# FerrisMind/candle-video

Measured on AMD Instinct MI355X. Metric: frames/sec end-to-end LTX-Video-2B 512x768x97; DiT step ms; VAE decode ms, higher is better.
Workload: dtype bf16; 1 GPU; LTX-Video-0.9.8-2B-distilled 512x768x97, 7 steps (configs.rs:223-240), untiled VAE decode; preset=0.9.8-2b-distilled, denoise_steps=7, parallelism=replicas x1 (no data-path collective)

## Files before the change

### candle-video_amd/csrc/capi_ops.hip

```cpp
#include "conv3d.h"
#include "../../include/ltxhip_ops.h"
#include "../../include/ltxhip_upsampler_st.h"
#include "../../include/ltxhip_stg.h"

static inline int dtc(int d) { return d == 1 ? LTX_DT_BF16 : LTX_DT_F32; }

extern "C" int ltx_op_linear(const void* x, const void* w, const void* bias, void* y, int M, int N, int K, int dtype, int epi,
                             const void* resid, const float* gate, int rows_per_batch, ltx_stream stream) {
    if (!x || !w || !y) LTX_FAIL(LTX_ERR_ARG, "ltx_op_linear: null tensor");
    if (epi < 0 || epi > 3) LTX_FAIL(LTX_ERR_ARG, "ltx_op_linear: epi must be 0..3");
    if ((epi == 2 || epi == 3) && !resid) LTX_FAIL(LTX_ERR_ARG, "ltx_op_linear: residual epilogue needs resid");
    if (epi == 2 && (!gate || rows_per_batch < 1)) LTX_FAIL(LTX_ERR_ARG, "ltx_op_linear: gated epilogue needs gate");
    GemmArgs g; g.A = x; g.W = w; g.C = y; g.bias = bias; g.resid = resid; g.gate = gate;
    g.M = M; g.N = N; g.K = K; g.lda = K; g.ldc = N; g.ldr = N; g.rows_per_batch = rows_per_batch > 0 ? rows_per_batch : 1; g.gate_stride = N;
    return ltx_launch_gemm(g, dtc(dtype), epi, (hipStream_t)stream);
}

extern "C" int64_t ltx_op_ring_packed_bytes(int N, int K) { return (int64_t)ltx_ring_packed_bytes(N, K); }
extern "C" int ltx_op_ring_pack(const void* w, int N, int K, void* out, ltx_stream stream) { return ltx_pack_ring_weights(w, N, K, out, (hipStream_t)stream); }
extern "C" int ltx_op_linear_packed(const void* x, const void* w, const void* w_packed, const void* bias, void* y, int M, int N, int K, int epi,
                                    const void* resid, const float* gate, int rows_per_batch, ltx_stream stream) {
    if (!x || !w || !w_packed || !y) LTX_FAIL(LTX_ERR_ARG, "ltx_op_linear_packed: null tensor");
    if (epi < 0 || epi > 3) LTX_FAIL(LTX_ERR_ARG, "ltx_op_linear_packed: epi must be 0..3");
    if ((epi == 2 || epi == 3) && !resid) LTX_FAIL(LTX_ERR_ARG, "ltx_op_linear_packed: residual epilogue needs resid");
// ... 305 lines not shown
        a.B = B; a.Sq = Sq; a.Sk = Sk; a.heads = heads; a.hd = 64; a.scale = scale; a.bias = (const float*)bc; a.k_count = (const int*)cnt;
        a.p_out = p_out; a.ldp = heads * KP;
        if (q_rowsq) { a.q_rowsq = q_rowsq; a.q_rowsq_n = q_rowsq_n; a.q_rowsq_D = D; a.q_rowsq_eps = q_rowsq_eps; }
        rc = ltx_launch_attention(a, LTX_DT_BF16, s);
    }
    if (rc == LTX_OK && counts_out && hipMemcpyAsync(counts_out, cnt, (size_t)B * 4, hipMemcpyDeviceToDevice, s) != hipSuccess) rc = LTX_ERR_HIP;
    const hipError_t e = hipStreamSynchronize(s);
    free_all();
    if (rc != LTX_OK) return rc;
    if (e != hipSuccess) { ltx_set_error(hipGetErrorString(e)); return LTX_ERR_HIP; }
    return LTX_OK;
}

extern "C" int ltx_op_attention_prescaled(const void* q, const void* k, const void* v, void* o, int B, int Sq, int Sk, int heads, int hd,
                                          int ldq, int ldk, int ldv, int ldo, ltx_stream stream) {
    if (!q || !k || !v || !o) LTX_FAIL(LTX_ERR_ARG, "ltx_op_attention_prescaled: null tensor");
    AttnArgs a; a.q = q; a.k = k; a.v = v; a.o = o; a.ldq = ldq; a.ldk = ldk; a.ldv = ldv; a.ldo = ldo;
    a.B = B; a.Sq = Sq; a.Sk = Sk; a.heads = heads; a.hd = hd; a.scale = 1.0f; a.q_prescaled = 1;
    return ltx_launch_attention(a, LTX_DT_BF16, (hipStream_t)stream);
}

namespace {
int conv_common(const void* x, const void* w, const void* bias, int wdtype, void* y, const void* resid,
                int B, int T, int H, int W, int Cin, int Cout, int causal, int dtype, int epi, int mode, int post, hipStream_t s, const PostNorm* pn = nullptr) {
    if (!x || !w || !bias || !y) LTX_FAIL(LTX_ERR_ARG, "conv: null tensor");
    const int dt = dtc(dtype), pad_t = causal ? 2 : 1;
    const Dims d{B, T, H, W};
    ConvW cw; cw.cin = Cin; cw.cout = Cout;
    if (pn) {
        if (B < 1 || T < 1 || H < 1 || W < 1 || Cin < 1 || Cout < 1) LTX_FAIL(LTX_ERR_ARG, "conv: empty problem");
        ConvW raw = cw; raw.w = const_cast<void*>(w); raw.b = const_cast<void*>(bias);
        GemmArgs g = conv_args(raw, d, pad_t, epi, pn); g.A = x; g.C = y;
        GemmRoute r;
        LTX_TRY(ltx_gemm_route(g, dt, epi, nullptr, false, &r));
        if (const char* why = ltx_gemm_route_refusal(g, r)) LTX_FAIL(LTX_ERR_ARG, why);
    }
    return conv3d_unpacked(dt, pad_t, cw, w, bias, dtc(wdtype), mode, x, y, d, epi, resid, post, s, pn);
}
}

extern "C" int ltx_op_conv3d(const void* x, const void* w, const void* bias, int wdtype, void* y, const void* resid,
                             int B, int T, int H, int W, int Cin, int Cout, int causal, int dtype, ltx_stream stream) {
    return conv_common(x, w, bias, wdtype, y, resid, B, T, H, W, Cin, Cout, causal, dtype, resid ? EPI_RESID : EPI_BIAS, LTX_PERM_NONE, 0, (hipStream_t)stream);
}
extern "C" int ltx_op_conv3d_norm(const void* x, const void* w, const void* bias, int wdtype, void* y, const float* scale, const float* shift, int mod_stride,
                                  float eps, int act, int B, int T, int H, int W, int Cin, int Cout, int causal, int dtype, ltx_stream stream) {
    if ((scale == nullptr) != (shift == nullptr)) LTX_FAIL(LTX_ERR_ARG, "ltx_op_conv3d_norm: scale and shift come together (both null: no modulation)");
    if (scale && mod_stride < Cout) LTX_FAIL(LTX_ERR_ARG, "ltx_op_conv3d_norm: mod_stride is the row stride of scale / shift, at least Cout");
    if (act != 0 && act != 1) LTX_FAIL(LTX_ERR_ARG, "ltx_op_conv3d_norm: act must be 0 (none) or 1 (SiLU)");
    if (!(eps >= 0.f)) LTX_FAIL(LTX_ERR_ARG, "ltx_op_conv3d_norm: eps must not be negative");
    PostNorm pn; pn.on = 1; pn.eps = eps; pn.act = act; pn.scale = scale; pn.shift = shift; pn.mod_stride = scale ? mod_stride : 0;
    return conv_common(x, w, bias, wdtype, y, nullptr, B, T, H, W, Cin, Cout, causal, dtype, EPI_BIAS, LTX_PERM_NONE, 0, (hipStream_t)stream, &pn);
}
extern "C" int ltx_op_upsample3d(const void* x, const void* w, const void* bias, int wdtype, void* y,
                                 int B, int T, int H, int W, int Cin, int Cout, int causal, int residual, int dtype, ltx_stream stream) {
    if (Cout % 8 != 0 || Cin % 8 != 0) LTX_FAIL(LTX_ERR_ARG, "upsample3d: channels must be multiples of 8");
    return conv_common(x, w, bias, wdtype, y, residual ? x : nullptr, B, T, H, W, Cin, Cout, causal, dtype, EPI_D2S, LTX_PERM_D2S, 0, (hipStream_t)stream);
}
extern "C" int ltx_op_conv3d_shuffle(const void* x, const void* w, const void* bias, int wdtype, void* y,
                                     int B, int F, int H, int W, int Cin, int O, int st, int ss, int dtype, ltx_stream stream) {
    if (!x || !w || !bias || !y) LTX_FAIL(LTX_ERR_ARG, "ltx_op_conv3d_shuffle: null tensor");
    if (!((st == 2 && ss == 1) || (st == 2 && ss == 2) || (st == 1 && ss == 2))) LTX_FAIL(LTX_ERR_ARG, "ltx_op_conv3d_shuffle: the factors (st, ss) are (2,1), (2,2) or (1,2)");
    if ((dtype != 0 && dtype != 1) || (wdtype != 0 && wdtype != 1)) LTX_FAIL(LTX_ERR_ARG, "ltx_op_conv3d_shuffle: bad dtype");
    const int nsub = st * ss * ss;
    if (B < 1 || F < 1 || H < 1 || W < 1 || F > (1 << 29) || H > (1 << 29) || W > (1 << 29)) LTX_FAIL(LTX_ERR_ARG, "ltx_op_conv3d_shuffle: bad shape");
    if (Cin < 8 || Cin % 8 != 0 || O < 4 * nsub || O % (4 * nsub) != 0) LTX_FAIL(LTX_ERR_ARG, "ltx_op_conv3d_shuffle: Cin must be a multiple of 8 and O a multiple of 4 x the sub-pixel count");
    if ((int64_t)B * (2 * F + 1) * (2 * H) * (2 * W) * std::max(Cin, O) > (1LL << 40)) LTX_FAIL(LTX_ERR_ARG, "ltx_op_conv3d_shuffle: shape too large");
    ConvW cw; cw.cin = Cin; cw.cout = O; cw.nsub = nsub;
    return conv3d_unpacked(dtc(dtype), 1, cw, w, bias, dtc(wdtype), LTX_PERM_D2S, x, y, Dims{B, F + 2, H, W}, EPI_D2S_G, nullptr, 0, (hipStream_t)stream);
}
extern "C" int ltx_op_conv_out_unpatchify(const void* x, const void* w, const void* bias, int wdtype, float* y,
                                          int B, int T, int H, int W, int Cin, int Cout, int causal, int postprocess, int dtype, ltx_stream stream) {
    if (Cout % 16 != 0) LTX_FAIL(LTX_ERR_ARG, "conv_out: Cout must be a multiple of 16 (patch 4x4)");
    return conv_common(x, w, bias, wdtype, y, nullptr, B, T, H, W, Cin, Cout, causal, dtype, EPI_UNPATCH, LTX_PERM_UNPATCH, postprocess, (hipStream_t)stream);
}

extern "C" int ltx_op_blend(const float* a, float* b, int BC, int at, int ah, int aw, int bt, int bh, int bw, int dim, int blend_extent, ltx_stream stream) {
    if (!a || !b || dim < 2 || dim > 4) LTX_FAIL(LTX_ERR_ARG, "ltx_op_blend: bad argument");
    const int ad[3] = {at, ah, aw}, bd[3] = {bt, bh, bw};
    BlendArgs ba; ba.a = a; ba.b = b; ba.dst = b; ba.BC = BC;
// ... 57 lines not shown
```

### candle-video_amd/csrc/conv_halo.hip

```cpp
#include <type_traits>
#include "gemm_common.h"
#include "options.h"

#ifndef HALO_WIDE_EPI
#define HALO_WIDE_EPI 1
#endif
#ifndef HALO_LOADERS
#define HALO_LOADERS 4
#endif
#ifndef HALO_PABL
#define HALO_PABL 0
#endif
#ifndef HALO_ABL
#define HALO_ABL 0
#endif

#ifdef HALO_TRACE
__device__ unsigned long long g_halo_trace[16384 * 8];
extern "C" int ltx_dbg_halo_trace(unsigned long long* out, int n) { return hipMemcpyFromSymbol(out, HIP_SYMBOL(g_halo_trace), (size_t)n * 8) == hipSuccess ? 0 : -1; }
#define HSTAMP(i) do { if (threadIdx.x == 0 && blockIdx.x < 16384) g_halo_trace[blockIdx.x * 8 + (i)] = __builtin_amdgcn_s_memrealtime(); } while (0)
#define HCYC(i) do { if (threadIdx.x == 0 && blockIdx.x < 16384) g_halo_trace[blockIdx.x * 8 + (i)] = __builtin_amdgcn_s_memtime(); } while (0)
#else
#define HSTAMP(i) do { } while (0)
#define HCYC(i) do { } while (0)
#endif

namespace {

constexpr int ROWB = 128;
constexpr int PH = 16, PW = 16, HW = PW + 2, HROWS = (PH + 2) * HW;
constexpr int A_PIECES = (HROWS + 7) / 8;
constexpr int A_STAGE = A_PIECES * 1024;
constexpr uint32_t OOB = 0x80000000u;
template <int I, int N, typename F> __device__ __forceinline__ void sfor_h(F&& f) {
    if constexpr (I < N) { f(std::integral_constant<int, I>{}); sfor_h<I + 1, N>(f); }
}

__device__ __forceinline__ int swz_h(int row, int chunk) { return row * ROWB + ((chunk ^ ((row >> 1) & 7)) << 4); }

extern __shared__ __attribute__((aligned(16))) unsigned char halo_smem[];

template <int BN, int WGM, int WGN, int EPI, bool PIPE>
__global__ __launch_bounds__(WGM * WGN * 64) void conv_halo_kernel(const GemmArgs g) {
    constexpr int NW = WGM * WGN, BM = PH * PW, WM = BM / WGM, WN = BN / WGN, FM = WM / 16, FN = BN == 64 ? 3 : WN / 16;
    static_assert((NW == 8 || (NW == 4 && PIPE)) && WM % 16 == 0 && WN % 16 == 0, "wave layout");
    constexpr int NTHR = NW * 64;
    constexpr int NL = (HALO_LOADERS == 4 && (BN == 128 || (BN == 64 && PIPE))) ? 4 : NW;
    constexpr int AJ = (A_PIECES + NL - 1) / NL, BJ = BN / (8 * NL);
    constexpr int B_STAGE = BN * ROWB;
    constexpr int A_ST = PIPE ? AJ * NL * 1024 : A_STAGE;
    static_assert(!PIPE || (NL == 4 && (BN == 128 || BN == 64)), "pipelined form: four loader waves, 128-wide tile (or conv_out's 64-wide one)");
    unsigned char* Abuf = halo_smem;
    unsigned char* Bbuf = halo_smem + 2 * A_ST;
    HSTAMP(0);
#ifndef HALO_NO_KERNARG_BATCH
    asm volatile("" :: "s"(g.A), "s"(g.W), "s"(g.C), "s"(g.bias), "s"(g.resid), "s"(g.N), "s"(g.K), "s"(g.Cin), "s"(g.T), "s"(g.H), "s"(g.Wd), "s"(g.ntaps), "s"(g.pad_t),
                 "s"(g.ldc), "s"(g.ldr), "s"(gridDim.x));
#endif

    const int tid = threadIdx.x, lane = tid & 63, wave = __builtin_amdgcn_readfirstlane(tid >> 6);
    const int wm = wave / WGN, wn = wave % WGN;
    const int lwave = wave & (NL - 1);
    const bool loader = wave < NL;
// ... 277 lines not shown
#pragma unroll
            for (int fm = 0; fm < FM; ++fm) {
                if (fm + 1 < FM) __builtin_amdgcn_sched_group_barrier(0x100, 1, 0);
                __builtin_amdgcn_sched_group_barrier(0x008, FN, 0);
            }
        }
        asm volatile("s_waitcnt vmcnt(0)" ::: "memory");
        __syncthreads();
    };
    for (int grp = 0; grp < G; ++grp) {
        const int p = grp & 1;
        step(grp, std::integral_constant<int, 0>{}, p);
        step(grp, std::integral_constant<int, 1>{}, p ^ 1);
        step(grp, std::integral_constant<int, 2>{}, p);
        step(grp, std::integral_constant<int, 3>{}, p ^ 1);
        step(grp, std::integral_constant<int, 4>{}, p);
        step(grp, std::integral_constant<int, 5>{}, p ^ 1);
        step(grp, std::integral_constant<int, 6>{}, p);
        step(grp, std::integral_constant<int, 7>{}, p ^ 1);
        step(grp, std::integral_constant<int, 8>{}, p);
    }

    }
    constexpr bool WIDE = HALO_WIDE_EPI && (EPI == EPI_BIAS || EPI == EPI_RESID);
    if constexpr (WIDE) {
        if (g.wide_epi) {
            constexpr int CPR = BN / 8, XM = 15, RPP = 64 / CPR;
            const int64_t frame_row0 = ((int64_t)b * g.T + t) * g.H * g.Wd;
            const __amdgpu_buffer_rsrc_t rr = __builtin_amdgcn_make_buffer_rsrc(
                const_cast<bf16_t*>(reinterpret_cast<const bf16_t*>(g.resid ? g.resid : g.C) + frame_row0 * g.ldr), 0, (int)OOB, 0x00020000);
            auto row_m = [&](int row, bool& inside) {
                const int y = y0 + (row >> 4), x = x0 + (row & 15);
                inside = y < g.H && x < g.Wd;
                return ((b * g.T + t) * g.H + y) * g.Wd + x;
            };
            if constexpr (EPI == EPI_RESID) {
                for (int pi = wave; pi < BM / RPP; pi += NW) {
                    const int row = pi * RPP + lane / CPR, pc = lane % CPR;
                    const int lc = pc ^ (row & XM);
                    bool inside; const int m = row_m(row, inside);
                    dma(rr, inside ? (uint32_t)((((int64_t)m - frame_row0) * g.ldr + n0 + lc * 8) * 2) : OOB, 0u, halo_smem + pi * 1024);
                }
                asm volatile("s_waitcnt vmcnt(0)" ::: "memory");
            }
            float bias4[FN][4];
#pragma unroll
            for (int fn = 0; fn < FN; ++fn) {
#pragma unroll
                for (int i = 0; i < 4; ++i) bias4[fn][i] = 0.f;
            }
// ... 18 lines not shown
                        float r[4];
                        load4<bf16_t>(reinterpret_cast<const bf16_t*>(slot), r);
#pragma unroll
                        for (int i = 0; i < 4; ++i) v[i] += r[i];
                    }
                    store4<bf16_t>(reinterpret_cast<bf16_t*>(slot), v);
                }
            }
            __syncthreads();
            bf16_t* Cb = reinterpret_cast<bf16_t*>(g.C);
            float pn_sc[8], pn_sh[8];
            bool pn_mod = false;
            if constexpr (EPI == EPI_BIAS) {
                if (g.pn_on && g.pn_scale) {
                    pn_mod = true;
                    const int c0 = tid % CPR;
                    const f32x4* scp = reinterpret_cast<const f32x4*>(g.pn_scale + (int64_t)b * g.pn_mod_stride + c0 * 8);
                    const f32x4* shp = reinterpret_cast<const f32x4*>(g.pn_shift + (int64_t)b * g.pn_mod_stride + c0 * 8);
                    const f32x4 s0 = scp[0], s1 = scp[1], h0 = shp[0], h1 = shp[1];
#pragma unroll
                    for (int j = 0; j < 4; ++j) { pn_sc[j] = 1.0f + s0[j]; pn_sc[4 + j] = 1.0f + s1[j]; pn_sh[j] = h0[j]; pn_sh[4 + j] = h1[j]; }
                }
            }
            for (int id = tid; id < BM * CPR; id += NTHR) {
                const int row = id / CPR, c = id - row * CPR;
                bool inside; const int m = row_m(row, inside);
                Chunk16 cc; cc.u = *reinterpret_cast<const u32x4*>(halo_smem + row * (CPR * 16) + ((c ^ (row & XM)) << 4));
                if constexpr (EPI == EPI_BIAS) {
                    if (g.pn_on) {
                        float f[8]; chunk_to_f32<bf16_t>(cc, f);
                        float ss = 0.f;
#pragma unroll
                        for (int j = 0; j < 8; ++j) ss += f[j] * f[j];
#pragma unroll
                        for (int o = CPR / 2; o > 0; o >>= 1) ss += __shfl_xor(ss, o);
                        const float rinv = __builtin_amdgcn_rsqf(ss * (1.0f / (float)BN) + g.pn_eps);
#pragma unroll
                        for (int j = 0; j < 8; ++j) {
                            float n = f[j] * rinv;
                            if (pn_mod) n = n * pn_sc[j] + pn_sh[j];
                            if (g.pn_act == 1) n = silu_f(n);
                            f[j] = n;
                        }
                        f32_to_chunk<bf16_t>(f, cc);
                    }
                }
                if (!inside) continue;
                *reinterpret_cast<u32x4*>(Cb + (int64_t)m * g.ldc + n0 + c * 8) = cc.u;
            }
#ifdef HALO_TRACE
            HSTAMP(3); asm volatile("s_waitcnt vmcnt(0)" ::: "memory"); HSTAMP(4);
            if (threadIdx.x == 0 && blockIdx.x < 16384) { unsigned hw; asm volatile("s_getreg_b32 %0, hwreg(HW_REG_HW_ID)" : "=s"(hw)); g_halo_trace[blockIdx.x * 8 + 7] = hw; }
#endif
            return;
        }
    }
    if constexpr (EPI == EPI_S2D) {
        float bias4[FN][4];
#pragma unroll
        for (int fn = 0; fn < FN; ++fn) {
#pragma unroll
            for (int i = 0; i < 4; ++i) bias4[fn][i] = 0.f;
        }
        if (g.bias) {
#pragma unroll
            for (int fn = 0; fn < FN; ++fn) {
                int nb = n0 + wn * WN + fn * 16 + 4 * fq; nb = nb < g.N ? nb : g.N - 4;
                load4<bf16_t>(reinterpret_cast<const bf16_t*>(g.bias) + nb, bias4[fn]);
            }
        }
        const int npass = (t == 0 && g.s2_st > 1) ? 2 : 1;
        for (int pass = 0; pass < npass; ++pass) {
// ... 18 lines not shown
                    for (int i = 0; i < 4; ++i) v[i] = acc[fm][fn][i] + bias4[fn][i];
                    s2d_store<bf16_t>(g, b, t, y, x, nb, pass, v, res[fn]);
                }
            }
        }
    } else if constexpr (EPI == EPI_D2S || EPI == EPI_UNPATCH || EPI == EPI_BIAS || EPI == EPI_D2S_G) {
        float bias4[FN][4];
#pragma unroll
        for (int fn = 0; fn < FN; ++fn) {
            const int nb = n0 + wn * WN + fn * 16 + 4 * fq;
#pragma unroll
            for (int i = 0; i < 4; ++i) bias4[fn][i] = 0.f;
        }
        if (g.bias) {
#pragma unroll
            for (int fn = 0; fn < FN; ++fn) {
                int nb = n0 + wn * WN + fn * 16 + 4 * fq; nb = nb < g.N ? nb : g.N - 4;
                load4<bf16_t>(reinterpret_cast<const bf16_t*>(g.bias) + nb, bias4[fn]);
            }
        }
        const bool d2s_res = EPI == EPI_D2S && g.resid != nullptr;
        GemmArgs gs = g; gs.bias = nullptr; gs.resid = nullptr;
        constexpr int FC = FM * FN > 16 ? 2 : FM;
#pragma unroll
        for (int f0 = 0; f0 < FM; f0 += FC) {
            bf16_t raw[FC][FN][4];
            if constexpr (EPI == EPI_D2S) {
                if (d2s_res) {
                    const int nsub = g.d2s_sp ? 4 : 8;
#pragma unroll
                    for (int fc = 0; fc < FC; ++fc) {
                        int y = y0 + wm * FM + f0 + fc, x = x0 + frow;
                        y = y < g.H ? y : g.H - 1; x = x < g.Wd ? x : g.Wd - 1;
                        const int m = ((b * g.T + t) * g.H + y) * g.Wd + x;
                        const bf16_t* xr = reinterpret_cast<const bf16_t*>(g.resid) + (int64_t)m * g.Cin;
#pragma unroll
                        for (int fn = 0; fn < FN; ++fn) {
                            int nb = n0 + wn * WN + fn * 16 + 4 * fq; nb = nb < g.N ? nb : g.N - 4;
                            const int sidx = nb / g.Cf, co = nb - sidx * g.Cf;
#pragma unroll
                            for (int i = 0; i < 4; ++i) raw[fc][fn][i] = xr[((co + i) % g.Cr) * nsub + sidx];
                        }
                    }
                }
            }
#pragma unroll
            for (int fc = 0; fc < FC; ++fc) {
                const int fm = f0 + fc;
                const int y = y0 + wm * FM + fm, x = x0 + frow;
                if (y >= g.H || x >= g.Wd) continue;
                const int m = ((b * g.T + t) * g.H + y) * g.Wd + x;
#pragma unroll
                for (int fn = 0; fn < FN; ++fn) {
                    const int nb = n0 + wn * WN + fn * 16 + 4 * fq;
                    if (nb >= g.N) continue;
                    float v[4];
#pragma unroll
                    for (int i = 0; i < 4; ++i) v[i] = acc[fm][fn][i] + bias4[fn][i];
                    if constexpr (EPI == EPI_D2S) {
                        if (d2s_res) {
#pragma unroll
                            for (int i = 0; i < 4; ++i) v[i] += to_f32(raw[fc][fn][i]);
                        }
                    }
                    epilogue<bf16_t, EPI>(gs, m, nb, v);
                }
            }
        }
    } else {
#pragma unroll
    for (int fm = 0; fm < FM; ++fm) {
        const int y = y0 + wm * FM + fm, x = x0 + frow;
        if (y >= g.H || x >= g.Wd) continue;
        const int m = ((b * g.T + t) * g.H + y) * g.Wd + x;
#pragma unroll
        for (int fn = 0; fn < FN; ++fn) {
            const int nb = n0 + wn * WN + fn * 16 + 4 * fq;
            if (nb >= g.N) continue;
            float v[4] = {acc[fm][fn][0], acc[fm][fn][1], acc[fm][fn][2], acc[fm][fn][3]};
            epilogue<bf16_t, EPI>(g, m, nb, v);
        }
    }
    }
}

bool halo_wide_epi(const GemmArgs& g) {
    return ltx_opt().gemm_wide_epi && g.ldc % 8 == 0 && ((uintptr_t)g.C & 15) == 0 &&
           (!g.resid || (g.ldr % 8 == 0 && ((uintptr_t)g.resid & 15) == 0 && (double)g.H * g.Wd * g.ldr * 2.0 < 2147483648.0));
}

template <int BN, int WGM, int WGN, int EPI, bool PIPE = false>
int launch_halo(const GemmArgs& g, hipStream_t s) {
    constexpr int smem = PIPE ? 2 * 44 * 1024 + 3 * BN * ROWB : 2 * A_STAGE + 2 * BN * ROWB;
    static std::atomic<unsigned long long> attr_devs{0};
    auto kern = conv_halo_kernel<BN, WGM, WGN, EPI, PIPE>;
    LTX_TRY(ltx_set_max_dyn_smem(attr_devs, reinterpret_cast<const void*>(kern), smem));
    const int tiles = g.B * g.T * cdiv(g.H, PH) * cdiv(g.Wd, PW) * cdiv(g.N, BN);
    GemmArgs ga = g;
    ga.wide_epi = halo_wide_epi(g);
    if (g.pn_on && (!ga.wide_epi || BN != g.N || !ltx_conv_halo_norm_ok(g, EPI))) LTX_FAIL(LTX_ERR_ARG, "conv_halo: the fused output norm needs the wide bias epilogue and BN == N");
    LTX_LAUNCH_TIMED(kern, dim3((unsigned)tiles), dim3(WGM * WGN * 64), smem, s, ga);
    LTX_CHECK_LAUNCH();
    return LTX_OK;
}

template <int BN, int WGM, int WGN, bool PIPE = false>
int launch_halo_epi(const GemmArgs& g, int epi, hipStream_t s) {
    switch (epi) {
        case EPI_BIAS: return launch_halo<BN, WGM, WGN, EPI_BIAS, PIPE>(g, s);
        case EPI_RESID: return launch_halo<BN, WGM, WGN, EPI_RESID, PIPE>(g, s);
        case EPI_D2S: return launch_halo<BN, WGM, WGN, EPI_D2S, PIPE>(g, s);
        case EPI_S2D: return launch_halo<BN, WGM, WGN, EPI_S2D, PIPE>(g, s);
        case EPI_D2S_G: return launch_halo<BN, WGM, WGN, EPI_D2S_G, PIPE>(g, s);
    }
    LTX_FAIL(LTX_ERR_ARG, "conv_halo: unsupported epilogue");
}

}

bool ltx_conv_halo_eligible(const GemmArgs& g, int epi, int bn) {
    if (!g.conv || g.ntaps != 27 || g.kh != 3 || g.kw != 3) return false;
    if (g.Cin % 64 != 0 || g.K != g.Cin) return false;
// ... 38 lines not shown
```

### candle-video_amd/csrc/options.cpp

```cpp
#include "options.h"
#include <atomic>
#include <cstdio>
#include <cstdlib>
#include <cstring>
#include <map>
#include <mutex>
#include <string>
#include "errors.h"

namespace {
std::mutex g_mu;
LtxOptions g_opt;
std::atomic<bool> g_loaded{false};
std::map<std::string, int> g_exp;

struct ListBit { const char* name; unsigned bit; };
const ListBit kFam[] = {{"asm16", LTX_FAM_ASM16}, {"ring", LTX_FAM_RING}, {"p8", LTX_FAM_P8}, {"halo", LTX_FAM_HALO}, {"halo_out", LTX_FAM_HALO_OUT}, {"big", LTX_FAM_BIG}};
const ListBit kAttn[] = {{"q64", LTX_ATTN_Q64}, {"q128", LTX_ATTN_Q128}, {"cross", LTX_ATTN_CROSS}, {"pipe", LTX_ATTN_PIPE}};

template <size_t N> bool parse_list(const char* v, const ListBit (&tab)[N], unsigned* out) {
    unsigned bits = 0;
    std::string s(v ? v : "");
    size_t p = 0;
    while (p < s.size()) {
        size_t q = s.find('+', p); if (q == std::string::npos) q = s.size();
        const std::string item = s.substr(p, q - p);
        bool ok = item.empty();
        for (const auto& t : tab) if (item == t.name) { bits |= t.bit; ok = true; }
        if (!ok) return false;
        p = q + 1;
    }
    *out = bits;
    return true;
}

struct IntField { const char* name; int LtxOptions::*field; };
const IntField kInts[] = {
    {"gemm_tune", &LtxOptions::gemm_tune}, {"gemm_wide_epi", &LtxOptions::gemm_wide_epi}, {"gemm_trace", &LtxOptions::gemm_trace},
    {"attn_q64_big", &LtxOptions::attn_q64_big}, {"vae_tile_batch", &LtxOptions::vae_tile_batch}, {"prof_kernel_events", &LtxOptions::prof_kernel_events}, {"ff2_defer", &LtxOptions::ff2_defer},
    {"gemm_splitk", &LtxOptions::gemm_splitk}, {"q2_fold", &LtxOptions::q2_fold}, {"norm_presum", &LtxOptions::norm_presum}, {"norm_lean", &LtxOptions::norm_lean},
    {"xattn_compact", &LtxOptions::xattn_compact}, {"xattn_fold_vo", &LtxOptions::xattn_fold_vo}, {"dense_qkv", &LtxOptions::dense_qkv}, {"vae_fuse_norm", &LtxOptions::vae_fuse_norm}, {"t5_attn_mfma", &LtxOptions::t5_attn_mfma}, {"guidance_batch", &LtxOptions::guidance_batch}, {"norm_fold", &LtxOptions::norm_fold}, {"norm_fold_copies", &LtxOptions::norm_fold_copies}, {"attn_q64_stream", &LtxOptions::attn_q64_stream},
};

bool set_one(LtxOptions& o, const std::string& key, const char* value) {
    static const LtxOptions dflt;
    for (const auto& f : kInts) if (key == f.name) {
        if (!value) { o.*(f.field) = dflt.*(f.field); return true; }
        char* end = nullptr; const long v = strtol(value, &end, 10);
        if (end == value || *end) return false;
        o.*(f.field) = (int)v; return true;
    }
    if (key == "gemm_plan") {
        if (!value) { o.gemm_plan[0] = 0; return true; }
        if (strlen(value) >= sizeof(o.gemm_plan)) return false;
        strcpy(o.gemm_plan, value); return true;
    }
    if (key == "gemm_off") return value ? parse_list(value, kFam, &o.gemm_off) : (o.gemm_off = 0, true);
    if (key == "attn_off") return value ? parse_list(value, kAttn, &o.attn_off) : (o.attn_off = 0, true);
    if (key.rfind("x_", 0) == 0) {
        if (!value) { g_exp.erase(key); return true; }
        char* end = nullptr; const long v = strtol(value, &end, 10);
// ... 81 lines not shown
```

### candle-video_amd/csrc/options.h

```cpp
#pragma once

enum { LTX_FAM_ASM16 = 1, LTX_FAM_RING = 2, LTX_FAM_P8 = 4, LTX_FAM_HALO = 8, LTX_FAM_HALO_OUT = 16, LTX_FAM_BIG = 32 };
enum { LTX_ATTN_Q64 = 1, LTX_ATTN_Q128 = 2, LTX_ATTN_CROSS = 4, LTX_ATTN_PIPE = 8 };

struct LtxOptions {
    int gemm_tune = 1;
    char gemm_plan[40] = {0};
    unsigned gemm_off = 0;
    int gemm_wide_epi = 1;
    int gemm_trace = 0;
    int attn_q64_big = -1;
    int vae_tile_batch = 0;
    int prof_kernel_events = 1;
    int ff2_defer = 1;
    int gemm_splitk = 1;
    int q2_fold = 1;
    int norm_presum = 1;
    int norm_lean = 1;
    int xattn_compact = 1;
    int xattn_fold_vo = 1;
    int attn_q64_stream = 0;
    int norm_fold = 2;
    int norm_fold_copies = 10;
    int guidance_batch = 1;
    int dense_qkv = 1;
    int vae_fuse_norm = 1;
    int t5_attn_mfma = 1;
    unsigned attn_off = 0;
};

const LtxOptions& ltx_opt();
int ltx_exp_lookup(const char* name, int dflt);
// ... 6 lines not shown
```

### candle-video_amd/ltxhip/__init__.py

```python
from __future__ import annotations

import ctypes as C
import os
from dataclasses import dataclass, field
from typing import Dict, List, Optional, Sequence, Tuple

import torch

_HERE = os.path.dirname(os.path.abspath(__file__))
_LIB_PATH = os.environ.get("LTXHIP_LIB") or os.path.join(os.path.dirname(_HERE), "libltxhip.so")

if not os.path.exists(_LIB_PATH):
    raise ImportError(
        f"ltxhip: {_LIB_PATH} is missing — build it with `make -C candle-video_amd` "
        "(or `python -c 'import __graft_entry__ as g; g.build()'`). There is no CPU fallback.")
lib = C.CDLL(_LIB_PATH)

LTX_F32, LTX_BF16 = 0, 1


class LtxError(RuntimeError):
    pass


# ... 85 lines not shown
    "ltx_op_linear_fold_out": [_vp, _vp, _vp, _vp, _vp, _vp, _vp, _i, _i, _i, _i, _i, _vp, _vp, _i, _vp],
    "ltx_op_linear_fold_in": [_vp, _vp, _vp, _vp, _i, _i, _f, _vp, _i, _i, _i, _i, _i, _i, _vp],
    "ltx_op_linear_fold_ok": [_i, _i, _i, _i, _i, _i, _i, _i],
    "ltx_op_shift_gemv": [_vp, _vp, _vp, _i, _i, _i, _i, _vp, _i, _vp],
    "ltx_op_mod_scale": [_vp, _vp, _i, _vp, _i, _i64, _i, _i, _vp], "ltx_op_scale_cols": [_vp, _vp, _vp, _i64, _i, _i, _vp],
    "ltx_op_linear_split_factor": [_i, _i, _i], "ltx_op_linear_deferred": [_vp, _vp, _vp, _i, _i, _i, _vp],
    "ltx_op_rownorm_deferred": [_vp, _i, _vp, _vp, _vp, _i, _vp, _vp, _i64, _i, _i, _f, _vp, _vp, _i64, _i, _i, _vp],
    "ltx_op_attention_compact": [_vp, _vp, _vp, _vp, _i, _i, _i, _i, _i, _i, _i, _i, _i, _f, _vp, _vp, _i, _i, _f, _vp, _vp],
    "ltx_op_attention_rowsq": [_vp, _vp, _vp, _vp, _i, _i, _i, _i, _i, _i, _i, _i, _i, _f, _vp, _vp, _i, _i, _f, _vp],
    "ltx_op_rownorm": [_vp, _vp, _i64, _i, _i, _f, _vp, _vp, _vp, _i64, _i, _i, _i, _vp],
    "ltx_op_qknorm_rope": [_vp, _i64, _i, _i, _vp, _f, _vp, _vp, _i, _vp],
    "ltx_op_qknorm_rope_segs": [_vp, _i64, _i, _i, _i, _i64, _vp, _vp, _vp, _f, _vp, _vp, _f, _i, _vp],
    "ltx_op_xattn_fold_route": [_i, _i, _i, _i, _i, _i, _i, C.POINTER(C.c_int)], "ltx_op_xattn_fold_kp": [C.POINTER(C.c_int), _i, C.POINTER(C.c_int)],
    "ltx_op_xattn_fold_build": [_vp, _vp, _vp, _i, _i, _i, _i, _vp, _vp, _vp],
    "ltx_op_attention_probs": [_vp, _vp, _vp, _i, _i, _i, _i, _i, _f, _vp, _vp, _i, _f, _vp, _vp],
    "ltx_op_norm_route": [_i64, _i, _i, _i, _i, _i, _i64, _i, _i, C.c_char_p, _i], "ltx_op_qknorm_route": [_i64, _i, _i, C.c_char_p, _i],
    "ltx_op_rope_table": [_vp, _vp, _vp, _i, _i, _i, _i, _i, _vp, _vp],
    "ltx_op_timestep_embedding": [_vp, _i, _i, _f, _i, _vp, _vp],
    "ltx_op_attention": [_vp, _vp, _vp, _vp, _i, _i, _i, _i, _i, _i, _i, _i, _i, _f, _vp, _i, _vp],
    "ltx_op_attention_prescaled": [_vp, _vp, _vp, _vp, _i, _i, _i, _i, _i, _i, _i, _i, _i, _vp],
    "ltx_op_conv3d": [_vp, _vp, _vp, _i, _vp, _vp, _i, _i, _i, _i, _i, _i, _i, _i, _vp],
    "ltx_op_conv3d_norm": [_vp, _vp, _vp, _i, _vp, _vp, _vp, _i, _f, _i, _i, _i, _i, _i, _i, _i, _i, _i, _vp],
    "ltx_op_upsample3d": [_vp, _vp, _vp, _i, _vp, _i, _i, _i, _i, _i, _i, _i, _i, _i, _vp],
    "ltx_op_conv_out_unpatchify": [_vp, _vp, _vp, _i, _vp, _i, _i, _i, _i, _i, _i, _i, _i, _i, _vp],
    "ltx_op_blend": [_vp, _vp, _i, _i, _i, _i, _i, _i, _i, _i, _i, _vp],
    "ltx_op_downsample3d": [_vp, _vp, _vp, _i, _vp, _i, _i, _i, _i, _i, _i, _i, _i, _vp],
    "ltx_op_gemm_plan": [_i, _i, _i, _i, _i, _i, _i, _i, C.c_char_p, _i],
    "ltx_op_gemm_route": [_i, _i, _i, _i, _i, _i, _i, _i, _i, _i, _i, _i, C.c_char_p, _i],
    "ltx_op_dit_plan": [_i, _i, _i, _i, _i, _i, _i, _i, _i, C.POINTER(C.c_int64)],
    "ltx_t5_config_default": [_vp], "ltx_t5_create": [_vp, _vp, _sz, _i, _i, _vp], "ltx_t5_destroy": [_vp],
    "ltx_t5_forward": [_vp, _vp, _i, _i, _i, _vp, _vp],
    "ltx_t5_create_from_gguf": [_vp, C.c_char_p, _i, _i, _vp], "ltx_t5_forward_masked": [_vp, _vp, _vp, _i, _i, _i, _vp, _vp],
    "ltx_gguf_open": [C.c_char_p, _vp], "ltx_gguf_close": [_vp], "ltx_gguf_count": [_vp], "ltx_gguf_find": [_vp, C.c_char_p],
    "ltx_gguf_tensor": [_vp, _sz, _vp, _vp, _vp, _vp, _vp, _vp], "ltx_gguf_type_info": [_i, _vp, _vp],
    "ltx_gguf_dequantize": [_i, _vp, _i, _i64, _i, _vp, _vp],
    "ltx_video_to_rgb8": [_vp, _i, _i, _i, _i, _vp, _vp], "ltx_write_png": [C.c_char_p, _vp, _i, _i],
    "ltx_save_frames_png": [_vp, _i, _i, _i, _i, C.c_char_p, _vp, _vp],
    "ltx_write_gif": [C.c_char_p, _vp, _i, _i, _i, _i, _i], "ltx_save_video_gif": [_vp, _i, _i, _i, _i, C.c_char_p, _vp],
    "ltx_preset_count": [], "ltx_preset_name": [_i], "ltx_preset_get": [C.c_char_p, _vp], "ltx_pipeline_params_from_preset": [_vp, _vp],
    "ltx_weights_detect_format": [C.c_char_p], "ltx_weights_remap_key": [C.c_char_p, C.c_char_p, _sz],
    "ltx_weights_is_transformer_key": [C.c_char_p], "ltx_weights_is_vae_key": [C.c_char_p],
    "ltx_name_mapper_create": [], "ltx_name_mapper_destroy": [_vp], "ltx_name_mapper_add": [_vp, _i, C.c_char_p, C.c_char_p],
    "ltx_name_mapper_has_mapping": [_vp, C.c_char_p], "ltx_name_mapper_map": [_vp, C.c_char_p, C.c_char_p, _sz],
    "ltx_weights_validate_names": [_vp, _sz, _vp, _sz, _vp, _vp],
    "ltx_safetensors_open": [C.c_char_p, _vp], "ltx_safetensors_close": [_vp], "ltx_safetensors_count": [_vp],
    "ltx_safetensors_tensor": [_vp, _sz, _vp, _vp, _vp, _vp, _vp, _vp],
# ... 1988 lines not shown
        ms = 0
        if scale is not None:
            for t in (scale, shift):
                if t.dtype != torch.float32 or tuple(t.shape) != (B, Cout) or t.stride(1) != 1:
                    raise LtxError(f"conv3d_norm: scale / shift must be f32 [{B}, {Cout}] with dense rows")
            ms = scale.stride(0) if B > 1 else max(scale.stride(0), Cout)
            if B > 1 and shift.stride(0) != ms:
                raise LtxError("conv3d_norm: scale and shift must share one row stride")
        y = torch.empty(B, T, H, W, Cout, dtype=x_cl.dtype, device=x_cl.device)
        _check(lib.ltx_op_conv3d_norm(_ptr(x_cl.contiguous()), _ptr(w.contiguous()), _ptr(bias.to(w.dtype).contiguous()), _dt(w.dtype), _ptr(y),
                                      _ptr(scale), _ptr(shift), ms, C.c_float(eps), act, B, T, H, W, Cin, Cout, int(causal), _dt(x_cl.dtype), _stream()))
        return y

    @staticmethod
    def upsample3d(x_cl, w, bias, causal=False, residual=True):
        B, T, H, W, Cin = x_cl.shape
        Cout = w.shape[0]
        y = torch.empty(B, 2 * T - 1, 2 * H, 2 * W, Cout // 8, dtype=x_cl.dtype, device=x_cl.device)
        _check(lib.ltx_op_upsample3d(_ptr(x_cl.contiguous()), _ptr(w.contiguous()), _ptr(bias.to(w.dtype).contiguous()), _dt(w.dtype), _ptr(y),
                                     B, T, H, W, Cin, Cout, int(causal), int(residual), _dt(x_cl.dtype), _stream()))
        return y

    @staticmethod
    def conv3d_shuffle(x_cl, w, bias, st, ss, out=None):
        x = x_cl.contiguous()
        B, Ft, H, W, Cin = x.shape
        F = Ft - 2
        O = w.shape[0]
        nsub = st * ss * ss
        shape = (B, (2 * F - 1 if st == 2 else F) + 2, ss * H, ss * W, O // max(nsub, 1))
        if out is None:
            out = torch.empty(shape, dtype=x.dtype, device=x.device)
        elif tuple(out.shape) != shape or out.dtype != x.dtype or not out.is_contiguous():
            raise LtxError(f"conv3d_shuffle: out must be a contiguous {shape} tensor of the input's dtype")
        _check(lib.ltx_op_conv3d_shuffle(_ptr(x), _ptr(w.contiguous()), _ptr(bias.to(w.dtype).contiguous()), _dt(w.dtype), _ptr(out),
                                         B, F, H, W, Cin, O, int(st), int(ss), _dt(x.dtype), _stream()))
        return out

    @staticmethod
    def pixel_shuffle_guarded(x_cl, out=None):
        x = x_cl.contiguous()
        B, Ft, H, W, C4 = x.shape
        if out is None:
            out = torch.empty(B, Ft, 2 * H, 2 * W, C4 // 4, dtype=x.dtype, device=x.device)
        _check(lib.ltx_op_pixel_shuffle_guarded(_ptr(x), _ptr(out), B, Ft - 2, H, W, C4 // 4, _dt(x.dtype), _stream()))
        return out
# ... 82 lines not shown
```

### include/ltxhip_ops.h

```cpp
#ifndef LTXHIP_OPS_H
#define LTXHIP_OPS_H
#include "ltxhip.h"
#ifdef __cplusplus
extern "C" {
#endif

int ltx_op_linear(const void* x, const void* w, const void* bias, void* y, int M, int N, int K, int dtype, int epi,
                  const void* resid, const float* gate, int rows_per_batch, ltx_stream stream);

int64_t ltx_op_ring_packed_bytes(int N, int K);
int ltx_op_ring_pack(const void* w, int N, int K, void* out, ltx_stream stream);
int ltx_op_linear_packed(const void* x, const void* w, const void* w_packed, const void* bias, void* y, int M, int N, int K, int epi,
                         const void* resid, const float* gate, int rows_per_batch, ltx_stream stream);
int ltx_op_linear_rowsq(const void* x, const void* w, const void* bias, void* y, float* rowsq, int M, int N, int K, int dtype, int epi,
                        const void* resid, const float* gate, int rows_per_batch, ltx_stream stream);
int ltx_op_rowsq(const void* x, int64_t rows, int N, int ld, float* rowsq, int dtype, ltx_stream stream);

int ltx_op_linear_fold_out(const void* x, const void* w, const void* bias, void* y, void* y2, float* rowsq, const float* scale2, int scale2_stride,
                           int M, int N, int K, int epi, const void* resid, const float* gate, int rows_per_batch, ltx_stream stream);
int ltx_op_linear_fold_in(const void* x, const void* w, void* y, const float* rs_sq, int rs_n, int rs_D, float eps, const float* cvec, int cvec_stride,
                          int M, int N, int K, int epi, int rows_per_batch, ltx_stream stream);
int ltx_op_linear_fold_ok(int M, int N, int K, int epi, int consumer, int rs_n, int vec_stride, int rows_per_batch);
int ltx_op_shift_gemv(const void* w, const void* bias, const float* shift, int shift_stride, int B, int N, int K, float* cvec, int cvec_stride, ltx_stream stream);
int ltx_op_mod_scale(const void* h, const float* scale, int scale_stride, void* y, int B, int64_t rows_per_batch, int D, int dtype, ltx_stream stream);
// ... 37 lines not shown
int ltx_op_attention_rowsq(const void* q, const void* k, const void* v, void* o, int B, int Sq, int Sk, int heads, int hd,
                           int ldq, int ldk, int ldv, int ldo, float scale, const float* key_bias,
                           const float* q_rowsq, int q_rowsq_n, int q_rowsq_D, float q_rowsq_eps, ltx_stream stream);
int ltx_op_attention_compact(const void* q, const void* k, const void* v, void* o, int B, int Sq, int Sk, int heads, int hd,
                             int ldq, int ldk, int ldv, int ldo, float scale, const float* key_bias,
                             const float* q_rowsq, int q_rowsq_n, int q_rowsq_D, float q_rowsq_eps, int* counts_out, ltx_stream stream);
int ltx_op_xattn_fold_route(int dtype, int head_dim, int heads, int D, int KP, int B, int compact, int* fold);
int ltx_op_xattn_fold_kp(const int* counts_host, int B, int* KP);
int ltx_op_xattn_fold_build(const void* v, const float* key_bias, const void* wo, int B, int K, int heads, int KP, void* vo, int* counts_out, ltx_stream stream);
int ltx_op_attention_probs(const void* q, const void* k, void* p_out, int B, int Sq, int Sk, int heads, int KP, float scale, const float* key_bias,
                           const float* q_rowsq, int q_rowsq_n, float q_rowsq_eps, int* counts_out, ltx_stream stream);
int ltx_op_attention_prescaled(const void* q, const void* k, const void* v, void* o, int B, int Sq, int Sk, int heads, int hd,
                               int ldq, int ldk, int ldv, int ldo, ltx_stream stream);

int ltx_op_conv3d(const void* x, const void* w, const void* bias, int wdtype, void* y, const void* resid,
                  int B, int T, int H, int W, int Cin, int Cout, int causal, int dtype, ltx_stream stream);

int ltx_op_conv3d_norm(const void* x, const void* w, const void* bias, int wdtype, void* y, const float* scale, const float* shift, int mod_stride,
                       float eps, int act, int B, int T, int H, int W, int Cin, int Cout, int causal, int dtype, ltx_stream stream);

int ltx_op_upsample3d(const void* x, const void* w, const void* bias, int wdtype, void* y,
                      int B, int T, int H, int W, int Cin, int Cout, int causal, int residual, int dtype, ltx_stream stream);

int ltx_op_downsample3d(const void* x, const void* w, const void* bias, int wdtype, void* y,
                        int B, int T, int H, int W, int Cin, int Cout, int down_type, int dtype, ltx_stream stream);

int ltx_op_conv_out_unpatchify(const void* x, const void* w, const void* bias, int wdtype, float* y,
                               int B, int T, int H, int W, int Cin, int Cout, int causal, int postprocess, int dtype, ltx_stream stream);

int ltx_op_blend(const float* a, float* b, int BC, int at, int ah, int aw, int bt, int bh, int bw, int dim, int blend_extent, ltx_stream stream);

int ltx_op_gemm_plan(int M, int N, int K, int conv, int ntaps, int T, int H, int W, char* name, int cap);

enum { LTX_ROUTE_PN = 1,
       LTX_ROUTE_DEFER = 2,
       LTX_ROUTE_FOLD_IN = 4,
       LTX_ROUTE_FOLD_OUT = 8 };
int ltx_op_gemm_route(int M, int N, int K, int conv, int ntaps, int B, int T, int H, int W, int epi, int dtype, int flags, char* name, int cap);

enum { LTX_DIT_PLAN_FIELDS = 13 };
int ltx_op_dit_plan(int heads, int head_dim, int model_dtype, int io_dtype, int B, int S, int K, int G, int skip_mask, int64_t* out);

#ifdef __cplusplus
}
#endif
#endif
// ... 1 lines not shown
```

Before: 547.3 frames/sec.

## Stage conv depth-to-space output through LDS for wide coalesced stores; vectorize fused norm

```diff
diff --git a/candle-video_amd/csrc/capi_ops.hip b/candle-video_amd/csrc/capi_ops.hip
--- a/candle-video_amd/csrc/capi_ops.hip
+++ b/candle-video_amd/csrc/capi_ops.hip
@@ -351,11 +351,11 @@
 
 namespace {
 int conv_common(const void* x, const void* w, const void* bias, int wdtype, void* y, const void* resid,
-                int B, int T, int H, int W, int Cin, int Cout, int causal, int dtype, int epi, int mode, int post, hipStream_t s, const PostNorm* pn = nullptr) {
+                int B, int T, int H, int W, int Cin, int Cout, int causal, int dtype, int epi, int mode, int post, hipStream_t s, const PostNorm* pn = nullptr, int nsub = 8) {
     if (!x || !w || !bias || !y) LTX_FAIL(LTX_ERR_ARG, "conv: null tensor");
     const int dt = dtc(dtype), pad_t = causal ? 2 : 1;
     const Dims d{B, T, H, W};
-    ConvW cw; cw.cin = Cin; cw.cout = Cout;
+    ConvW cw; cw.cin = Cin; cw.cout = Cout; cw.nsub = nsub;
     if (pn) {
         if (B < 1 || T < 1 || H < 1 || W < 1 || Cin < 1 || Cout < 1) LTX_FAIL(LTX_ERR_ARG, "conv: empty problem");
         ConvW raw = cw; raw.w = const_cast<void*>(w); raw.b = const_cast<void*>(bias);
@@ -385,6 +385,11 @@
                                  int B, int T, int H, int W, int Cin, int Cout, int causal, int residual, int dtype, ltx_stream stream) {
     if (Cout % 8 != 0 || Cin % 8 != 0) LTX_FAIL(LTX_ERR_ARG, "upsample3d: channels must be multiples of 8");
     return conv_common(x, w, bias, wdtype, y, residual ? x : nullptr, B, T, H, W, Cin, Cout, causal, dtype, EPI_D2S, LTX_PERM_D2S, 0, (hipStream_t)stream);
+}
+extern "C" int ltx_op_upsample3d_spatial(const void* x, const void* w, const void* bias, int wdtype, void* y,
+                                         int B, int T, int H, int W, int Cin, int Cout, int causal, int residual, int dtype, ltx_stream stream) {
+    if (Cout % 16 != 0 || Cin % 4 != 0) LTX_FAIL(LTX_ERR_ARG, "upsample3d_spatial: Cout must be a multiple of 16 and Cin of 4");
+    return conv_common(x, w, bias, wdtype, y, residual ? x : nullptr, B, T, H, W, Cin, Cout, causal, dtype, EPI_D2S, LTX_PERM_D2S, 0, (hipStream_t)stream, nullptr, 4);
 }
 extern "C" int ltx_op_conv3d_shuffle(const void* x, const void* w, const void* bias, int wdtype, void* y,
                                      int B, int F, int H, int W, int Cin, int O, int st, int ss, int dtype, ltx_stream stream) {
diff --git a/candle-video_amd/csrc/conv_halo.hip b/candle-video_amd/csrc/conv_halo.hip
--- a/candle-video_amd/csrc/conv_halo.hip
+++ b/candle-video_amd/csrc/conv_halo.hip
@@ -39,6 +39,18 @@
 __device__ __forceinline__ int swz_h(int row, int chunk) { return row * ROWB + ((chunk ^ ((row >> 1) & 7)) << 4); }
 
 extern __shared__ __attribute__((aligned(16))) unsigned char halo_smem[];
+
+template <int CTRL> __device__ __forceinline__ float dpp_add(float v) {
+    return v + __builtin_bit_cast(float, __builtin_amdgcn_update_dpp(0, __builtin_bit_cast(int, v), CTRL, 0xf, 0xf, false));
+}
+template <int CPR> __device__ __forceinline__ float halo_row_sum(float ss) {
+    static_assert(CPR == 16 || CPR == 32, "a voxel's row on 16 or 32 lanes");
+    if constexpr (CPR == 32) ss += __builtin_bit_cast(float, __builtin_amdgcn_ds_swizzle(__builtin_bit_cast(int, ss), 0x401F));
+    ss = dpp_add<0x128>(ss);
+    ss = dpp_add<0x124>(ss);
+    ss = dpp_add<0x4E>(ss);
+    return dpp_add<0xB1>(ss);
+}
 
 template <int BN, int WGM, int WGN, int EPI, bool PIPE>
 __global__ __launch_bounds__(WGM * WGN * 64) void conv_halo_kernel(const GemmArgs g) {
@@ -362,10 +374,29 @@
     }
 
     }
+    constexpr int CPR = BN / 8, XM = 15, ITERS = BM * CPR / NTHR, RPI = NTHR / CPR, NB = ITERS < 8 ? ITERS : 8;
+    const int rc = tid % CPR, rrow0 = tid / CPR;
+    const int ryy0 = y0 + (rrow0 >> 4), rxx = x0 + (rrow0 & 15);
+    auto lds_rows_out = [&](bf16_t* dst, int64_t dstep, bool col_ok, auto&& finish) {
+        static_assert(BM * CPR % NTHR == 0 && NTHR % CPR == 0 && RPI % 16 == 0 && ITERS % NB == 0, "row loop: whole patch rows per iteration, whole rounds");
+        const unsigned char* lsrc = halo_smem + rrow0 * (CPR * 16) + ((rc ^ (rrow0 & XM)) << 4);
+#pragma unroll 1
+        for (int i0 = 0; i0 < ITERS; i0 += NB) {
+            Chunk16 v[NB];
+#pragma unroll
+            for (int i = 0; i < NB; ++i) v[i].u = *reinterpret_cast<const u32x4*>(lsrc + (i0 + i) * (NTHR * 16));
+            finish(v);
+#pragma unroll
+            for (int i = 0; i < NB; ++i) asm volatile("" : "+v"(v[i].u));
+#pragma unroll
+            for (int i = 0; i < NB; ++i)
+                if (col_ok && ryy0 + (i0 + i) * (RPI / 16) < g.H) *reinterpret_cast<u32x4*>(dst + (i0 + i) * dstep) = v[i].u;
+        }
+    };
     constexpr bool WIDE = HALO_WIDE_EPI && (EPI == EPI_BIAS || EPI == EPI_RESID);
     if constexpr (WIDE) {
         if (g.wide_epi) {
-            constexpr int CPR = BN / 8, XM = 15, RPP = 64 / CPR;
+            constexpr int RPP = 64 / CPR;
             const int64_t frame_row0 = ((int64_t)b * g.T + t) * g.H * g.Wd;
             const __amdgpu_buffer_rsrc_t rr = __builtin_amdgcn_make_buffer_rsrc(
                 const_cast<bf16_t*>(reinterpret_cast<const bf16_t*>(g.resid ? g.resid : g.C) + frame_row0 * g.ldr), 0, (int)OOB, 0x00020000);
@@ -430,32 +461,61 @@
                     for (int j = 0; j < 4; ++j) { pn_sc[j] = 1.0f + s0[j]; pn_sc[4 + j] = 1.0f + s1[j]; pn_sh[j] = h0[j]; pn_sh[4 + j] = h1[j]; }
                 }
             }
-            for (int id = tid; id < BM * CPR; id += NTHR) {
-                const int row = id / CPR, c = id - row * CPR;
-                bool inside; const int m = row_m(row, inside);
-                Chunk16 cc; cc.u = *reinterpret_cast<const u32x4*>(halo_smem + row * (CPR * 16) + ((c ^ (row & XM)) << 4));
-                if constexpr (EPI == EPI_BIAS) {
-                    if (g.pn_on) {
-                        float f[8]; chunk_to_f32<bf16_t>(cc, f);
-                        float ss = 0.f;
-#pragma unroll
-                        for (int j = 0; j < 8; ++j) ss += f[j] * f[j];
-#pragma unroll
-                        for (int o = CPR / 2; o > 0; o >>= 1) ss += __shfl_xor(ss, o);
-                        const float rinv = __builtin_amdgcn_rsqf(ss * (1.0f / (float)BN) + g.pn_eps);
-#pragma unroll
-                        for (int j = 0; j < 8; ++j) {
-                            float n = f[j] * rinv;
-                            if (pn_mod) n = n * pn_sc[j] + pn_sh[j];
-                            if (g.pn_act == 1) n = silu_f(n);
-                            f[j] = n;
+            bf16_t* dst = Cb + (((int64_t)(b * g.T + t) * g.H + ryy0) * g.Wd + rxx) * g.ldc + n0 + rc * 8;
+            const int64_t dstep = (int64_t)(RPI / 16) * g.Wd * g.ldc;
+            auto out_rows = [&](auto&& finish) { lds_rows_out(dst, dstep, rxx < g.Wd, finish); };
+            auto norm_rows = [&](auto mod_c, auto act_c) {
+                constexpr bool MOD = decltype(mod_c)::value, ACT = decltype(act_c)::value;
+                typedef float f2 __attribute__((ext_vector_type(2)));
+                typedef __bf16 h2 __attribute__((ext_vector_type(2)));
+                f2 sc2[4], sh2[4];
+#pragma unroll
+                for (int k = 0; k < 4; ++k) { sc2[k] = (f2){pn_sc[2 * k], pn_sc[2 * k + 1]}; sh2[k] = (f2){pn_sh[2 * k], pn_sh[2 * k + 1]}; }
+                const float eps = g.pn_eps;
+                out_rows([&](Chunk16 (&v)[NB]) {
+                    float ss[NB];
+#pragma unroll
+                    for (int i = 0; i < NB; ++i) {
+                        float f[8]; chunk_to_f32<bf16_t>(v[i], f);
+                        float s = f[1] * f[1];
+                        s = __builtin_fmaf(f[0], f[0], s);
+#pragma unroll
+                        for (int j = 2; j < 8; ++j) s = __builtin_fmaf(f[j], f[j], s);
+                        ss[i] = s;
+                    }
+#pragma unroll
+                    for (int i = 0; i < NB; ++i) ss[i] = halo_row_sum<CPR>(ss[i]);
+#pragma unroll
+                    for (int i = 0; i < NB; ++i) {
+                        const float rinv = __builtin_amdgcn_rsqf(__builtin_fmaf(ss[i], 1.0f / (float)BN, eps));
+                        float f[8]; chunk_to_f32<bf16_t>(v[i], f);
+#pragma unroll
+                        for (int k = 0; k < 4; ++k) {
+                            f2 n = (f2){f[2 * k], f[2 * k + 1]} * (f2){rinv, rinv};
+                            if constexpr (MOD) n = __builtin_elementwise_fma(n, sc2[k], sh2[k]);
+                            if constexpr (ACT) {
+                                const f2 a = n * (f2){-1.4426950408889634f, -1.4426950408889634f};
+                                f2 d = {__builtin_amdgcn_exp2f(a[0]), __builtin_amdgcn_exp2f(a[1])};
+                                d = d + (f2){1.0f, 1.0f};
+                                n = n * (f2){__builtin_amdgcn_rcpf(d[0]), __builtin_amdgcn_rcpf(d[1])};
+                            }
+                            v[i].u[k] = __builtin_bit_cast(uint32_t, __builtin_convertvector(n, h2));
                         }
-                        f32_to_chunk<bf16_t>(f, cc);
                     }
-                }
-                if (!inside) continue;
-                *reinterpret_cast<u32x4*>(Cb + (int64_t)m * g.ldc + n0 + c * 8) = cc.u;
-            }
+                });
+            };
+            bool normed = false;
+            if constexpr (EPI == EPI_BIAS) {
+                if (g.pn_on) {
+                    normed = true;
+                    const bool act = g.pn_act == 1;
+                    if (pn_mod && act) norm_rows(std::true_type{}, std::true_type{});
+                    else if (pn_mod) norm_rows(std::true_type{}, std::false_type{});
+                    else if (act) norm_rows(std::false_type{}, std::true_type{});
+                    else norm_rows(std::false_type{}, std::false_type{});
+                }
+            }
+            if (!normed) out_rows([](Chunk16 (&)[NB]) {});
 #ifdef HALO_TRACE
             HSTAMP(3); asm volatile("s_waitcnt vmcnt(0)" ::: "memory"); HSTAMP(4);
             if (threadIdx.x == 0 && blockIdx.x < 16384) { unsigned hw; asm volatile("s_getreg_b32 %0, hwreg(HW_REG_HW_ID)" : "=s"(hw)); g_halo_trace[blockIdx.x * 8 + 7] = hw; }
@@ -520,6 +580,8 @@
         const bool d2s_res = EPI == EPI_D2S && g.resid != nullptr;
         GemmArgs gs = g; gs.bias = nullptr; gs.resid = nullptr;
         constexpr int FC = FM * FN > 16 ? 2 : FM;
+        auto frag_rows = [&](auto to_lds_c) {
+        constexpr bool TO_LDS = decltype(to_lds_c)::value;
 #pragma unroll
         for (int f0 = 0; f0 < FM; f0 += FC) {
             bf16_t raw[FC][FN][4];
@@ -561,10 +623,31 @@
                             for (int i = 0; i < 4; ++i) v[i] += to_f32(raw[fc][fn][i]);
                         }
                     }
-                    epilogue<bf16_t, EPI>(gs, m, nb, v);
-                }
-            }
-        }
+                    if constexpr (TO_LDS) {
+                        const int row = (wm * FM + fm) * 16 + frow, col = wn * WN + fn * 16 + 4 * fq;
+                        store4<bf16_t>(reinterpret_cast<bf16_t*>(halo_smem + row * (CPR * 16) + (((col >> 3) ^ (row & XM)) << 4) + ((col >> 2) & 1) * 8), v);
+                    } else {
+                        epilogue<bf16_t, EPI>(gs, m, nb, v);
+                    }
+                }
+            }
+        }
+        };
+        if constexpr (EPI == EPI_D2S && HALO_WIDE_EPI && BN >= 128) {
+            if (g.wide_epi) {
+                asm volatile("s_waitcnt vmcnt(0)" ::: "memory");
+                __syncthreads();
+                frag_rows(std::true_type{});
+                __syncthreads();
+                const int nb = n0 + rc * 8, sidx = nb / g.Cf, co = nb - sidx * g.Cf;
+                const int st = sidx >> 2, sh = (sidx >> 1) & 1, sw = sidx & 1;
+                const int to = g.d2s_sp ? t : 2 * t + st - 1;
+                const int64_t o = ((((int64_t)b * g.To + to) * g.Ho + (2 * ryy0 + sh)) * g.Wo + (2 * rxx + sw)) * g.Cf + co;
+                lds_rows_out(reinterpret_cast<bf16_t*>(g.C) + o, (int64_t)(RPI / 16) * 2 * g.Wo * g.Cf, to >= 0 && rxx < g.Wd, [](Chunk16 (&)[NB]) {});
+                return;
+            }
+        }
+        frag_rows(std::false_type{});
     } else {
 #pragma unroll
     for (int fm = 0; fm < FM; ++fm) {
@@ -585,6 +668,10 @@
 bool halo_wide_epi(const GemmArgs& g) {
     return ltx_opt().gemm_wide_epi && g.ldc % 8 == 0 && ((uintptr_t)g.C & 15) == 0 &&
            (!g.resid || (g.ldr % 8 == 0 && ((uintptr_t)g.resid & 15) == 0 && (double)g.H * g.Wd * g.ldr * 2.0 < 2147483648.0));
+}
+
+bool halo_wide_d2s(const GemmArgs& g) {
+    return ltx_opt().gemm_wide_epi && ltx_opt().conv_d2s_wide && g.Cf > 0 && g.Cf % 8 == 0 && ((uintptr_t)g.C & 15) == 0;
 }
 
 template <int BN, int WGM, int WGN, int EPI, bool PIPE = false>
@@ -595,7 +682,7 @@
     LTX_TRY(ltx_set_max_dyn_smem(attr_devs, reinterpret_cast<const void*>(kern), smem));
     const int tiles = g.B * g.T * cdiv(g.H, PH) * cdiv(g.Wd, PW) * cdiv(g.N, BN);
     GemmArgs ga = g;
-    ga.wide_epi = halo_wide_epi(g);
+    ga.wide_epi = EPI == EPI_D2S ? halo_wide_d2s(g) : halo_wide_epi(g);
     if (g.pn_on && (!ga.wide_epi || BN != g.N || !ltx_conv_halo_norm_ok(g, EPI))) LTX_FAIL(LTX_ERR_ARG, "conv_halo: the fused output norm needs the wide bias epilogue and BN == N");
     LTX_LAUNCH_TIMED(kern, dim3((unsigned)tiles), dim3(WGM * WGN * 64), smem, s, ga);
     LTX_CHECK_LAUNCH();
diff --git a/candle-video_amd/csrc/options.cpp b/candle-video_amd/csrc/options.cpp
--- a/candle-video_amd/csrc/options.cpp
+++ b/candle-video_amd/csrc/options.cpp
@@ -36,7 +36,7 @@
 
 struct IntField { const char* name; int LtxOptions::*field; };
 const IntField kInts[] = {
-    {"gemm_tune", &LtxOptions::gemm_tune}, {"gemm_wide_epi", &LtxOptions::gemm_wide_epi}, {"gemm_trace", &LtxOptions::gemm_trace},
+    {"gemm_tune", &LtxOptions::gemm_tune}, {"gemm_wide_epi", &LtxOptions::gemm_wide_epi}, {"conv_d2s_wide", &LtxOptions::conv_d2s_wide}, {"gemm_trace", &LtxOptions::gemm_trace},
     {"attn_q64_big", &LtxOptions::attn_q64_big}, {"vae_tile_batch", &LtxOptions::vae_tile_batch}, {"prof_kernel_events", &LtxOptions::prof_kernel_events}, {"ff2_defer", &LtxOptions::ff2_defer},
     {"gemm_splitk", &LtxOptions::gemm_splitk}, {"q2_fold", &LtxOptions::q2_fold}, {"norm_presum", &LtxOptions::norm_presum}, {"norm_lean", &LtxOptions::norm_lean},
     {"xattn_compact", &LtxOptions::xattn_compact}, {"xattn_fold_vo", &LtxOptions::xattn_fold_vo}, {"dense_qkv", &LtxOptions::dense_qkv}, {"vae_fuse_norm", &LtxOptions::vae_fuse_norm}, {"t5_attn_mfma", &LtxOptions::t5_attn_mfma}, {"guidance_batch", &LtxOptions::guidance_batch}, {"norm_fold", &LtxOptions::norm_fold}, {"norm_fold_copies", &LtxOptions::norm_fold_copies}, {"attn_q64_stream", &LtxOptions::attn_q64_stream},
diff --git a/candle-video_amd/csrc/options.h b/candle-video_amd/csrc/options.h
--- a/candle-video_amd/csrc/options.h
+++ b/candle-video_amd/csrc/options.h
@@ -8,6 +8,7 @@
     char gemm_plan[40] = {0};
     unsigned gemm_off = 0;
     int gemm_wide_epi = 1;
+    int conv_d2s_wide = 1;
     int gemm_trace = 0;
     int attn_q64_big = -1;
     int vae_tile_batch = 0;
diff --git a/candle-video_amd/ltxhip/__init__.py b/candle-video_amd/ltxhip/__init__.py
--- a/candle-video_amd/ltxhip/__init__.py
+++ b/candle-video_amd/ltxhip/__init__.py
@@ -131,6 +131,7 @@
     "ltx_op_conv3d": [_vp, _vp, _vp, _i, _vp, _vp, _i, _i, _i, _i, _i, _i, _i, _i, _vp],
     "ltx_op_conv3d_norm": [_vp, _vp, _vp, _i, _vp, _vp, _vp, _i, _f, _i, _i, _i, _i, _i, _i, _i, _i, _i, _vp],
     "ltx_op_upsample3d": [_vp, _vp, _vp, _i, _vp, _i, _i, _i, _i, _i, _i, _i, _i, _i, _vp],
+    "ltx_op_upsample3d_spatial": [_vp, _vp, _vp, _i, _vp, _i, _i, _i, _i, _i, _i, _i, _i, _i, _vp],
     "ltx_op_conv_out_unpatchify": [_vp, _vp, _vp, _i, _vp, _i, _i, _i, _i, _i, _i, _i, _i, _i, _vp],
     "ltx_op_blend": [_vp, _vp, _i, _i, _i, _i, _i, _i, _i, _i, _i, _vp],
     "ltx_op_downsample3d": [_vp, _vp, _vp, _i, _vp, _i, _i, _i, _i, _i, _i, _i, _i, _vp],
@@ -2165,6 +2166,15 @@
         return y
 
     @staticmethod
+    def upsample3d_spatial(x_cl, w, bias, causal=False, residual=True):
+        B, T, H, W, Cin = x_cl.shape
+        Cout = w.shape[0]
+        y = torch.empty(B, T, 2 * H, 2 * W, Cout // 4, dtype=x_cl.dtype, device=x_cl.device)
+        _check(lib.ltx_op_upsample3d_spatial(_ptr(x_cl.contiguous()), _ptr(w.contiguous()), _ptr(bias.to(w.dtype).contiguous()), _dt(w.dtype), _ptr(y),
+                                             B, T, H, W, Cin, Cout, int(causal), int(residual), _dt(x_cl.dtype), _stream()))
+        return y
+
+    @staticmethod
     def conv3d_shuffle(x_cl, w, bias, st, ss, out=None):
         x = x_cl.contiguous()
         B, Ft, H, W, Cin = x.shape
diff --git a/include/ltxhip_ops.h b/include/ltxhip_ops.h
--- a/include/ltxhip_ops.h
+++ b/include/ltxhip_ops.h
@@ -83,6 +83,9 @@
 int ltx_op_upsample3d(const void* x, const void* w, const void* bias, int wdtype, void* y,
                       int B, int T, int H, int W, int Cin, int Cout, int causal, int residual, int dtype, ltx_stream stream);
 
+int ltx_op_upsample3d_spatial(const void* x, const void* w, const void* bias, int wdtype, void* y,
+                              int B, int T, int H, int W, int Cin, int Cout, int causal, int residual, int dtype, ltx_stream stream);
+
 int ltx_op_downsample3d(const void* x, const void* w, const void* bias, int wdtype, void* y,
                         int B, int T, int H, int W, int Cin, int Cout, int down_type, int dtype, ltx_stream stream);
 
```

Result: no change. 549.2 frames/sec (median of 6 runs) (+0.3%).
